# Auxeno/diamond-ppo

Measured on NVIDIA B200. Metric: ppo_update_samples_per_s, higher is better.
Workload: dtype f32

## Files before the change

diamond-ppo_b200/csrc/api.cu:

```cuda
#include "common.cuh"
#include "heads.cuh"
#include "optim.cuh"
#include "gemm_tc.cuh"

char g_dppo_create_error[512] = "";

extern "C" int dppo_version(void) { return DPPO_VERSION; }

extern "C" const char* dppo_last_error(dppo_ctx* ctx) { return ctx ? ctx->err : g_dppo_create_error; }

extern "C" int dppo_create(dppo_ctx** out, int device)
{
    if (!out) return 1;
    *out = nullptr;
    int count = 0;
    cudaError_t e = cudaGetDeviceCount(&count);
    if (e != cudaSuccess || count == 0) {
        snprintf(g_dppo_create_error, sizeof(g_dppo_create_error),
                 "dppo_create: no CUDA device (%s); libdppo has no CPU fallback", cudaGetErrorString(e));
        return 2;
    }
    if (device < 0 || device >= count) {
        snprintf(g_dppo_create_error, sizeof(g_dppo_create_error), "dppo_create: device %d out of range (%d devices)", device, count);
        return 3;
    }
    cudaDeviceProp prop;
    e = cudaGetDeviceProperties(&prop, device);
    if (e != cudaSuccess) {
        snprintf(g_dppo_create_error, sizeof(g_dppo_create_error), "dppo_create: %s", cudaGetErrorString(e));
        return 4;
    }
    if (prop.major != 10) {
        snprintf(g_dppo_create_error, sizeof(g_dppo_create_error),
                 "dppo_create: device %d is sm_%d%d; libdppo embeds sm_100a code only (B200) and has no fallback", device,
                 prop.major, prop.minor);
        return 5;
    }
    dppo_ctx* c = new dppo_ctx();
    c->device = device;
    c->sm_count = prop.multiProcessorCount;
    c->cc_major = prop.major;
    c->cc_minor = prop.minor;
    c->err[0] = 0;
    c->use_tensor_cores = 3;
    c->gae_variant = 0;
    c->gae_inputs_settled = 0;
    c->tc_debug = 0;
    c->row_sweep = 31;
    c->tc_prefetch = 0;
    c->draw_base = nullptr;
    c->rows_dev = nullptr;
    c->launch_count = 0;
    c->tm_cache = nullptr;
    c->tm_cache_free = nullptr;
    *out = c;
    return 0;
}

extern "C" int dppo_destroy(dppo_ctx* ctx)
{
    if (ctx && ctx->tm_cache && ctx->tm_cache_free) ctx->tm_cache_free(ctx->tm_cache);
    delete ctx;
    return 0;
}

extern "C" int dppo_set_option(dppo_ctx* ctx, const char* name, int value)
{
    if (!ctx || !name) return 1;
    if (!strcmp(name, "tensor_cores")) { ctx->use_tensor_cores = value != 0 ? 3 : 0; return 0; }
    if (!strcmp(name, "row_sweep")) { ctx->row_sweep = value & 31; return 0; }
    if (!strcmp(name, "tc_prefetch")) { ctx->tc_prefetch = value & 7; return 0; }
    if (!strcmp(name, "gae_variant")) { ctx->gae_variant = value; return 0; }
    if (!strcmp(name, "tc_debug")) {
#ifdef DPPO_TIMING_SWITCHES
        ctx->tc_debug = value;
        return 0;
#else
        DPPO_FAIL(ctx, "dppo_set_option: 'tc_debug' needs a library built with -DDPPO_TIMING_SWITCHES (timing experiments only)");
#endif
    }
    if (!strcmp(name, "gae_inputs_settled")) { ctx->gae_inputs_settled = value < 0 ? 0 : value > 2 ? 2 : value; return 0; }
    DPPO_FAIL(ctx, "dppo_set_option: unknown option '%s'", name);
}

extern "C" int64_t dppo_launch_count(dppo_ctx* ctx) { return ctx ? ctx->launch_count : 0; }

extern "C" int dppo_count_launches(dppo_ctx* ctx, int64_t n)
{
    if (!ctx) return 1;
    ctx->launch_count += n;
    return 0;
}

extern "C" int dppo_device_info(dppo_ctx* ctx, int* sm_count, int* cc_major, int* cc_minor)
{
    if (!ctx) return 1;
    if (sm_count) *sm_count = ctx->sm_count;
    if (cc_major) *cc_major = ctx->cc_major;
    if (cc_minor) *cc_minor = ctx->cc_minor;
    return 0;
}

extern "C" int dppo_mlp_layout_compute(const dppo_mlp_desc* d, dppo_mlp_layout* L)
{
    if (!d || !L || d->obs_dim < 1 || d->hidden < 1 || d->act_dim < 1) return 1;
    const int64_t D = d->obs_dim, H = d->hidden, A = d->act_dim;
    int64_t o = 0;
    auto take = [&](int64_t n) { const int64_t at = o; o += align_up(n, 4); return at; };
    L->w1 = take(H * D); L->b1 = take(H);
    L->w2 = take(H * H); L->b2 = take(H);
    L->w3 = take(2 * H * H); L->b3 = take(2 * H);
    L->wa = take(A * H); L->ba = take(A);
    L->wc = take(H); L->bc = take(1);
    L->log_std = d->continuous ? take(A) : -1;
    L->total = o;
    return 0;
}

namespace {

struct WImages {
    unsigned char *w1f, *w2f, *w3f, *w3b, *w2b;
    int64_t bytes;
};

WImages carve_images(const dppo_mlp_desc* d, char* base)
{
    const int64_t D = d->obs_dim, H = d->hidden;
    WImages w;
    int64_t o = 0;
    auto take = [&](int64_t bytes) { unsigned char* p = reinterpret_cast<unsigned char*>(base + o); o += align_up(bytes, 1024); return p; };
    w.w1f = take(dppo_tc_image_bytes((int)H, (int)D));
    w.w2f = take(dppo_tc_image_bytes((int)H, (int)H));
    w.w3f = take(dppo_tc_image_bytes((int)(2 * H), (int)H));
    w.w3b = take(dppo_tc_image_bytes((int)H, (int)(2 * H)));
    w.w2b = take(dppo_tc_image_bytes((int)H, (int)H));
    w.bytes = o;
    return w;
}

struct TrainWs {
    float *h1, *h2, *h3, *d3, *d2, *d1, *xg;
    float *p3, *p2, *p1, *c2, *c1, *hp;
    int s3, s2, s1, tiles2, tiles1, head_blocks, head_stride;
    int t3, t2, t1;
    bool multi;
    float *zd, *pa, *ca;
    int sa, tiles_a;
    int64_t img_off;
    int64_t bytes;
};

TrainWs carve_train(const dppo_mlp_desc* d, int64_t M, int sm_count, char* base, bool gemm_heads = false)
{
    dppo_ctx fake = {}; fake.sm_count = sm_count;
    const int64_t D = d->obs_dim, H = d->hidden, A = d->act_dim;
    TrainWs w;
    int64_t o = 0;
    auto take = [&](int64_t floats) { float* p = reinterpret_cast<float*>(base + o); o += align_up(floats * 4, 256); return p; };
    w.h1 = take(M * H); w.h2 = take(M * H); w.h3 = take(M * 2 * H);
    w.d3 = take(M * 2 * H); w.d2 = take(M * H); w.d1 = take(M * H);
    w.xg = take(M * D);
    w.s3 = dppo_wgrad_splits(&fake, M, (int)(2 * H), (int)H);
    w.s2 = dppo_wgrad_splits(&fake, M, (int)H, (int)H);
    w.s1 = dppo_wgrad_splits(&fake, M, (int)H, (int)D);
    w.t3 = dppo_tc2_wgrad_supported(M, (int)(2 * H), (int)H) ? dppo_tc2_wgrad_splits(&fake, M, (int)(2 * H), (int)H) : 0;
    w.t2 = dppo_tc2_wgrad_supported(M, (int)H, (int)H) ? dppo_tc2_wgrad_splits(&fake, M, (int)H, (int)H) : 0;
    w.t1 = dppo_tc2_wgrad_supported(M, (int)H, (int)D) ? dppo_tc2_wgrad_splits(&fake, M, (int)H, (int)D) : 0;
    w.multi = w.t3 > 0 && w.t2 > 0 && w.t1 > 0 && H % 256 == 0;
    if (w.multi) {
        const int n1s[3] = {(int)(2 * H), (int)H, (int)H}, n2s[3] = {(int)H, (int)H, (int)D};
        int sp[3];
        dppo_tc2_wgrad_multi_splits(&fake, M, 3, n1s, n2s, sp);
        w.t3 = sp[0]; w.t2 = sp[1]; w.t1 = sp[2];
    }
    auto mx = [](int a, int b) { return a > b ? a : b; };
    w.p3 = take((int64_t)mx(w.s3, w.t3) * 2 * H * H);
    w.p2 = take((int64_t)mx(w.s2, w.t2) * H * H);
    w.p1 = take((int64_t)mx(w.s1, w.t1) * H * D);
    w.tiles2 = dppo_gemm_row_tiles(M, (int)H);
    w.tiles1 = dppo_gemm_row_tiles(M, (int)H);
    const int cparts = mx(dppo_tc3_colsum_rows(&fake, M, (int)H), w.tiles2);
    w.c2 = take((int64_t)cparts * H);
    w.c1 = take((int64_t)cparts * H);
    w.zd = w.pa = w.ca = nullptr;
    w.sa = w.tiles_a = 0;
    if (gemm_heads) {
        w.zd = take(M * A);
        w.sa = dppo_wgrad_splits(&fake, M, (int)A, (int)H);
        w.pa = take((int64_t)w.sa * A * H);
        w.tiles_a = dppo_gemm_row_tiles(M, (int)H);
        w.ca = take((int64_t)w.tiles_a * H);
        w.head_blocks = wide_loss_blocks(&fake, M, (int)H, (int)A);
        w.head_stride = wide_offsets((int)H, (int)A).total;
    } else {
        w.head_blocks = head_train_blocks(&fake, M, (int)H, (int)A);
        w.head_stride = (int)align_up(head_partial_floats((int)H, (int)A), 4);
    }
    w.hp = take((int64_t)w.head_blocks * w.head_stride);
    o = align_up(o, 1024);
    w.img_off = o;
    o += carve_images(d, nullptr).bytes;
    w.bytes = o;
    return w;
}

int current_sm_count()
{
    int dev = 0, sms = 148;
    if (cudaGetDevice(&dev) == cudaSuccess) cudaDeviceGetAttribute(&sms, cudaDevAttrMultiProcessorCount, dev);
    return sms > 0 ? sms : 148;
}

}

extern "C" int64_t dppo_mlp_workspace_bytes(const dppo_mlp_desc* d, int64_t rows, int training)
{
    if (!d || rows <= 0) return 0;
    const int64_t H = d->hidden;
    if (!training)
        return align_up(rows * H * 4, 256) * 2 + align_up(rows * 2 * H * 4, 256) + align_up(rows * (int64_t)d->obs_dim * 4, 256) + 1024 +
               carve_images(d, nullptr).bytes;
    int sms = current_sm_count();
    if (sms < 148) sms = 148;
    return carve_train(d, rows, sms, nullptr).bytes;
}

extern "C" int dppo_mlp_fused_heads_supported(const dppo_mlp_desc* d)
{
    return d && head_train_supported(d->hidden, d->act_dim) ? 1 : 0;
}

static bool gemm_heads_in_bound(const dppo_mlp_desc* d)
{
    return d->hidden >= 1 && d->hidden <= DPPO_GEMM_HEADS_MAX_HIDDEN && d->act_dim >= 1 && d->act_dim <= DPPO_GEMM_HEADS_MAX_ACT;
}

extern "C" int64_t dppo_mlp_gemm_heads_workspace_bytes(const dppo_mlp_desc* d, int64_t rows)
{
    if (!d || rows <= 0 || d->obs_dim < 1 || !gemm_heads_in_bound(d)) return 0;
    int sms = current_sm_count();
    if (sms < 148) sms = 148;
    return carve_train(d, rows, sms, nullptr, true).bytes;
}

extern "C" int dppo_mlp_forward(dppo_ctx* ctx, const dppo_mlp_desc* d, const float* params, const float* obs,
                                const int32_t* idx, int64_t rows, int heads, float* head_out, float* values, void* ws,
                                int64_t ws_bytes, void* stream)
{
    if (!ctx) return 1;
    if (!d || !params || !obs || rows <= 0) DPPO_FAIL(ctx, "mlp_forward: bad arguments");
    if ((heads & 3) == 0) DPPO_FAIL(ctx, "mlp_forward: heads mask selects nothing");
    if ((heads & 1) && !head_out) DPPO_FAIL(ctx, "mlp_forward: head_out is null");
    if ((heads & 2) && !values) DPPO_FAIL(ctx, "mlp_forward: values is null");
    dppo_mlp_layout L;
    if (dppo_mlp_layout_compute(d, &L)) DPPO_FAIL(ctx, "mlp_forward: bad descriptor");
    const int D = d->obs_dim, H = d->hidden, A = d->act_dim;
    cudaStream_t st = (cudaStream_t)stream;
    const int64_t img_bytes = align_up(carve_images(d, nullptr).bytes, 1024);
    char* base0 = (char*)ws;
    char* aligned = reinterpret_cast<char*>((reinterpret_cast<uintptr_t>(base0) + 1023) & ~(uintptr_t)1023);
    const int64_t head_room = (aligned - base0) + img_bytes;
    const bool tc_on = ctx->use_tensor_cores && ws_bytes > head_room + 3 * 256;
    WImages img = carve_images(d, aligned);
    char* base = tc_on ? aligned + img_bytes : base0;
    const int64_t avail = tc_on ? ws_bytes - head_room : ws_bytes;
    const int64_t per_row = (int64_t)4 * H * 4 + (idx ? (int64_t)D * 4 : 0);
    int64_t chunk = (avail - 4 * 256) / per_row;
    if (chunk > rows) chunk = rows;
    if (chunk < 1) DPPO_FAIL(ctx, "mlp_forward: workspace too small (%lld bytes, need >= %lld per row)", (long long)ws_bytes, (long long)per_row);
    float* h1 = (float*)base;
    float* h2 = (float*)(base + align_up(chunk * H * 4, 256));
    float* h3 = (float*)(base + 2 * align_up(chunk * H * 4, 256));
    float* xg = (float*)(base + 2 * align_up(chunk * H * 4, 256) + align_up(chunk * 2 * H * 4, 256));
    const bool actor = heads & 1, critic = heads & 2;
    const int sweep = ctx->row_sweep;
    const int hint = (sweep & 8) ? 2 : 0;
    const int64_t w3off = actor ? 0 : (int64_t)H * H;
    const int b3off = actor ? 0 : H;
    const int n3 = (actor && critic) ? 2 * H : H;
    const int64_t first = rows < chunk ? rows : chunk;
    const bool tc1 = tc_on && dppo_tc3_gemm_supported(first, H, D), tc2 = tc_on && dppo_tc3_gemm_supported(first, H, H),
               tc3 = tc_on && dppo_tc3_gemm_supported(first, n3, H);
    {
        PrepJobs jobs;
        jobs.n = 0;
        jobs.gather = GatherJob{nullptr, nullptr, nullptr, 0, 0};
        auto job = [&](bool on, const float* W, int rows_w, int cols_w, unsigned char* im) {
            if (on) { jobs.job[jobs.n].W = W; jobs.job[jobs.n].rows_w = rows_w; jobs.job[jobs.n].cols_w = cols_w;
                      jobs.job[jobs.n].transpose = 0; jobs.job[jobs.n].n_tile = 0; jobs.job[jobs.n].img = im; ++jobs.n; }
        };
        job(tc1, params + L.w1, H, D, img.w1f);
        job(tc2, params + L.w2, H, H, img.w2f);
        job(tc3, params + L.w3 + w3off, n3, H, img.w3f);
        if (dppo_tc_prep_weights_multi(ctx, jobs, st)) return 1;
    }
    for (int64_t r0 = 0; r0 < rows; r0 += chunk) {
        const int64_t n = rows - r0 < chunk ? rows - r0 : chunk;
        const float* x = idx ? obs : obs + r0 * D;
        const int32_t* rowsel = idx ? idx + r0 : nullptr;
        if (tc1 && dppo_tc3_gemm_supported(n, H, D)) {
            if (rowsel) {
                if (dppo_gather_rows_f32(ctx, obs, rowsel, xg, n, D, stream)) return 1;
                x = xg;
            }
            if (dppo_tc3_gemm(ctx, DPPO_EPI_BIAS_TANH, x, D, img.w1f, params + L.b1, nullptr, 0, h1, H, nullptr, n, H, D, hint, st)) return 1;
        } else if (dppo_gemm_nt(ctx, DPPO_EPI_BIAS_TANH, x, D, rowsel, params + L.w1, D, params + L.b1, h1, H, n, H, D, st)) return 1;
        if (tc2 && dppo_tc3_gemm_supported(n, H, H)) {
            if (dppo_tc3_gemm(ctx, DPPO_EPI_BIAS_TANH, h1, H, img.w2f, params + L.b2, nullptr, 0, h2, H, nullptr, n, H, H, (sweep & 1) | hint, st)) return 1;
        } else if (dppo_gemm_nt(ctx, DPPO_EPI_BIAS_TANH, h1, H, nullptr, params + L.w2, H, params + L.b2, h2, H, n, H, H, st)) return 1;
        if (tc3 && dppo_tc3_gemm_supported(n, n3, H)) {
            if (dppo_tc3_gemm(ctx, DPPO_EPI_BIAS_TANH, h2, H, img.w3f, params + L.b3 + b3off, nullptr, 0, h3, n3, nullptr, n, n3, H, hint, st)) return 1;
        } else if (dppo_gemm_nt(ctx, DPPO_EPI_BIAS_TANH, h2, H, nullptr, params + L.w3 + w3off, H, params + L.b3 + b3off, h3, n3, n, n3, H, st)) return 1;
        const float* ha = actor ? h3 : nullptr;
        const float* hc = critic ? (actor ? h3 + H : h3) : nullptr;
        if (launch_heads_forward(ctx, ha, hc, n3, params + L.wa, params + L.ba, params + L.wc, params + L.bc,
                                 head_out ? head_out + r0 * A : nullptr, values ? values + r0 : nullptr, n, H, A, (sweep >> 1) & 1, st)) return 1;
    }
    return 0;
}

static int mlp_grad_minibatch_impl(dppo_ctx* ctx, const char* what, bool gemm_heads, const dppo_mlp_desc* d, const float* params,
                                   float* grads, const float* obs, const void* actions, const float* old_log_probs, const float* adv,
                                   const float* returns, const double* adv_stats, const int32_t* idx, int64_t M, const dppo_hyper* hy,
                                   float* losses, void* ws, int64_t ws_bytes, void* stream)
{
    if (!ctx) return 1;
    if (!d || !params || !grads || !obs || !actions || !old_log_probs || !adv || !returns || !hy || !ws)
        DPPO_FAIL(ctx, "%s: null argument", what);
    if (M <= 0) DPPO_FAIL(ctx, "%s: empty minibatch", what);
    if (hy->advantage_norm && (!adv_stats || hy->adv_count < 2)) DPPO_FAIL(ctx, "%s: advantage_norm needs adv_stats and adv_count >= 2", what);
    dppo_mlp_layout L;
    if (dppo_mlp_layout_compute(d, &L)) DPPO_FAIL(ctx, "%s: bad descriptor", what);
    if (gemm_heads && !gemm_heads_in_bound(d))
        DPPO_FAIL(ctx, "%s: hidden %d / %d actions outside the GEMM-head bound (hidden <= %d, 1..%d actions)", what, d->hidden, d->act_dim,
                  DPPO_GEMM_HEADS_MAX_HIDDEN, DPPO_GEMM_HEADS_MAX_ACT);
    const int D = d->obs_dim, H = d->hidden, A = d->act_dim;
    TrainWs w = carve_train(d, M, ctx->sm_count, (char*)ws, gemm_heads);
    if (w.bytes > ws_bytes) DPPO_FAIL(ctx, "%s: workspace too small (%lld < %lld)", what, (long long)ws_bytes, (long long)w.bytes);
    cudaStream_t st = (cudaStream_t)stream;
    const float inv_m = 1.0f / (float)(hy->loss_denominator > 0 ? hy->loss_denominator : M);

    char* img_base = reinterpret_cast<char*>((reinterpret_cast<uintptr_t>((char*)ws + w.img_off) + 1023) & ~(uintptr_t)1023);
    const bool img_fits = (img_base - (char*)ws) + carve_images(d, nullptr).bytes <= ws_bytes;
    const bool tc_on = ctx->use_tensor_cores && img_fits;
    WImages img = carve_images(d, img_base);
    const bool g1 = tc_on && dppo_tc3_gemm_supported(M, H, D), g2 = tc_on && dppo_tc3_gemm_supported(M, H, H),
               g3 = tc_on && dppo_tc3_gemm_supported(M, 2 * H, H), gb3 = tc_on && dppo_tc3_gemm_supported(M, H, 2 * H), gb2 = g2;
    const bool wg3 = tc_on && w.t3 > 0, wg2 = tc_on && w.t2 > 0, wg1 = tc_on && w.t1 > 0;
    const int sweep = ctx->row_sweep;
    const int hint = (sweep & 8) ? 2 : 0;
    const float* x1 = obs;
    const int32_t* x1_idx = idx;
    bool gather_pending = idx && (g1 || wg1);
    if (gather_pending) { x1 = w.xg; x1_idx = nullptr; }
    {
        PrepJobs jobs;
        jobs.n = 0;
        jobs.gather = GatherJob{nullptr, nullptr, nullptr, 0, 0};
        auto job = [&](bool on, const float* W, int rows_w, int cols_w, int transpose, unsigned char* im) {
            if (on) { jobs.job[jobs.n].W = W; jobs.job[jobs.n].rows_w = rows_w; jobs.job[jobs.n].cols_w = cols_w;
                      jobs.job[jobs.n].transpose = transpose; jobs.job[jobs.n].n_tile = 0; jobs.job[jobs.n].img = im; ++jobs.n; }
        };
        job(g1, params + L.w1, H, D, 0, img.w1f);
        job(g2, params + L.w2, H, H, 0, img.w2f);
        job(g3, params + L.w3, 2 * H, H, 0, img.w3f);
        job(gb3, params + L.w3, 2 * H, H, 1, img.w3b);
        job(gb2, params + L.w2, H, H, 1, img.w2b);
        if (gather_pending && D % 4 == 0 && (reinterpret_cast<uintptr_t>(obs) & 15u) == 0 && (reinterpret_cast<uintptr_t>(w.xg) & 15u) == 0) {
            jobs.gather = GatherJob{reinterpret_cast<const float4*>(obs), idx, reinterpret_cast<float4*>(w.xg), M, D / 4};
            gather_pending = false;
        }
        if (dppo_tc_prep_weights_multi(ctx, jobs, st)) return 1;
    }
    if (gather_pending && dppo_gather_rows_f32(ctx, obs, idx, w.xg, M, D, stream)) return 1;

    if (g1) {
        if (dppo_tc3_gemm(ctx, DPPO_EPI_BIAS_TANH, x1, D, img.w1f, params + L.b1, nullptr, 0, w.h1, H, nullptr, M, H, D, hint, st)) return 1;
    } else if (dppo_gemm_nt(ctx, DPPO_EPI_BIAS_TANH, x1, D, x1_idx, params + L.w1, D, params + L.b1, w.h1, H, M, H, D, st)) return 1;
    if (g2) {
        if (dppo_tc3_gemm(ctx, DPPO_EPI_BIAS_TANH, w.h1, H, img.w2f, params + L.b2, nullptr, 0, w.h2, H, nullptr, M, H, H, (sweep & 1) | hint, st)) return 1;
    } else if (dppo_gemm_nt(ctx, DPPO_EPI_BIAS_TANH, w.h1, H, nullptr, params + L.w2, H, params + L.b2, w.h2, H, M, H, H, st)) return 1;
    if (g3) {
        if (dppo_tc3_gemm(ctx, DPPO_EPI_BIAS_TANH, w.h2, H, img.w3f, params + L.b3, nullptr, 0, w.h3, 2 * H, nullptr, M, 2 * H, H, hint, st)) return 1;
    } else if (dppo_gemm_nt(ctx, DPPO_EPI_BIAS_TANH, w.h2, H, nullptr, params + L.w3, H, params + L.b3, w.h3, 2 * H, M, 2 * H, H, st)) return 1;

    if (!gemm_heads) {
        HeadTrainArgs ha;
        ha.h3 = w.h3; ha.d3 = w.d3;
        ha.wa = params + L.wa; ha.ba = params + L.ba; ha.wc = params + L.wc; ha.bc = params + L.bc;
        ha.log_std = d->continuous ? params + L.log_std : nullptr;
        ha.idx = idx;
        ha.actions_i = d->continuous ? nullptr : (const int32_t*)actions;
        ha.actions_f = d->continuous ? (const float*)actions : nullptr;
        ha.old_logp = old_log_probs; ha.adv = adv; ha.ret = returns;
        ha.adv_stats = adv_stats; ha.adv_count = hy->adv_count; ha.advantage_norm = hy->advantage_norm;
        ha.M = M; ha.H = H; ha.A = A;
        ha.clip = hy->ppo_clip; ha.vw = hy->value_loss_weight; ha.beta = hy->entropy_beta; ha.inv_m = inv_m;
        ha.partials = w.hp; ha.partial_stride = w.head_stride;
        ha.rev = (sweep >> 1) & 1; ha.keep_d3 = (sweep >> 2) & 1; ha.h3_first = (sweep >> 3) & 1;
        if (launch_head_train_kernel(ctx, ha, d->continuous, w.head_blocks, st)) return 1;
    } else {
        if (dppo_gemm_nt(ctx, DPPO_EPI_BIAS, w.h3, 2 * H, nullptr, params + L.wa, H, params + L.ba, w.zd, A, M, A, H, st)) return 1;
        WideLossArgs la = {};
        la.z = w.zd; la.dz = w.zd;
        la.log_std = d->continuous ? params + L.log_std : nullptr;
        la.h3 = w.h3; la.d3 = w.d3; la.wc = params + L.wc; la.bc = params + L.bc;
        la.idx = idx;
        la.actions_i = d->continuous ? nullptr : (const int32_t*)actions;
        la.actions_f = d->continuous ? (const float*)actions : nullptr;
        la.old_logp = old_log_probs; la.adv = adv; la.ret = returns;
        la.adv_stats = adv_stats; la.adv_count = hy->adv_count; la.advantage_norm = hy->advantage_norm;
        la.M = M; la.H = H; la.A = A;
        la.clip = hy->ppo_clip; la.vw = hy->value_loss_weight; la.beta = hy->entropy_beta; la.inv_m = inv_m;
        la.partials = w.hp; la.partial_stride = w.head_stride;
        if (launch_wide_loss_train(ctx, la, d->continuous, w.head_blocks, st)) return 1;
        if (dppo_gemm_nn_tanh_bwd(ctx, w.zd, A, params + L.wa, H, w.h3, 2 * H, w.d3, 2 * H, w.ca, M, H, A, st)) return 1;
        if (dppo_wgrad(ctx, w.zd, A, w.h3, 2 * H, nullptr, w.pa, w.sa, M, A, H, st)) return 1;
    }

    int tiles2 = w.tiles2, tiles1 = w.tiles1;
    if (gb3) {
        tiles2 = dppo_tc3_colsum_parts(ctx, M, H);
        if (dppo_tc3_gemm(ctx, DPPO_EPI_TANH_BWD, w.d3, 2 * H, img.w3b, nullptr, w.h2, H, w.d2, H, w.c2, M, H, 2 * H, hint, st)) return 1;
    } else if (dppo_gemm_nn_tanh_bwd(ctx, w.d3, 2 * H, params + L.w3, H, w.h2, H, w.d2, H, w.c2, M, H, 2 * H, st)) return 1;
    if (gb2) {
        tiles1 = dppo_tc3_colsum_parts(ctx, M, H);
        if (dppo_tc3_gemm(ctx, DPPO_EPI_TANH_BWD, w.d2, H, img.w2b, nullptr, w.h1, H, w.d1, H, w.c1, M, H, H, sweep & 1, st)) return 1;
    } else if (dppo_gemm_nn_tanh_bwd(ctx, w.d2, H, params + L.w2, H, w.h1, H, w.d1, H, w.c1, M, H, H, st)) return 1;
    const int n3p = wg3 ? w.t3 : w.s3, n2p = wg2 ? w.t2 : w.s2, n1p = wg1 ? w.t1 : w.s1;
    if (w.multi && wg3 && wg2 && wg1) {
        const float* Ds[3] = {w.d3, w.d2, w.d1};
        const float* Hs[3] = {w.h2, w.h1, x1};
        float* Ps[3] = {w.p3, w.p2, w.p1};
        const int ldds[3] = {2 * H, H, H}, ldhs[3] = {H, H, D}, sps[3] = {w.t3, w.t2, w.t1}, n1s[3] = {2 * H, H, H}, n2s[3] = {H, H, D};
        if (dppo_tc2_wgrad_multi(ctx, 3, Ds, ldds, Hs, ldhs, Ps, sps, M, n1s, n2s, st)) return 1;
    } else {
    if (wg3) {
        if (dppo_tc2_wgrad(ctx, w.d3, 2 * H, w.h2, H, w.p3, w.t3, M, 2 * H, H, st)) return 1;
    } else if (dppo_wgrad(ctx, w.d3, 2 * H, w.h2, H, nullptr, w.p3, w.s3, M, 2 * H, H, st)) return 1;
    if (wg2) {
        if (dppo_tc2_wgrad(ctx, w.d2, H, w.h1, H, w.p2, w.t2, M, H, H, st)) return 1;
    } else if (dppo_wgrad(ctx, w.d2, H, w.h1, H, nullptr, w.p2, w.s2, M, H, H, st)) return 1;
    if (wg1) {
        if (dppo_tc2_wgrad(ctx, w.d1, H, x1, D, w.p1, w.t1, M, H, D, st)) return 1;
    } else if (dppo_wgrad(ctx, w.d1, H, x1, D, x1_idx, w.p1, w.s1, M, H, D, st)) return 1;
    }

    GradSegTable tab;
    int n = 0;
    auto seg = [&](int64_t dst, int64_t count, const float* src, int64_t stride, int nparts) {
        tab.seg[n].dst = dst; tab.seg[n].count = count; tab.seg[n].src = src; tab.seg[n].stride = stride;
        tab.seg[n].nparts = nparts; tab.seg[n].pad = 0; ++n;
    };
    seg(L.w1, (int64_t)H * D, w.p1, (int64_t)H * D, n1p);
    seg(L.b1, H, w.c1, H, tiles1);
    seg(L.w2, (int64_t)H * H, w.p2, (int64_t)H * H, n2p);
    seg(L.b2, H, w.c2, H, tiles2);
    seg(L.w3, (int64_t)2 * H * H, w.p3, (int64_t)2 * H * H, n3p);
    int off_dba, off_dwc, off_dbc, off_dls, off_loss;
    if (!gemm_heads) {
        const HeadOffsets ho = head_offsets(H, A);
        off_dba = ho.dba; off_dwc = ho.dwc; off_dbc = ho.dbc; off_dls = ho.dls; off_loss = ho.loss;
        seg(L.b3, 2 * H, w.hp + ho.b3, w.head_stride, w.head_blocks);
        seg(L.wa, (int64_t)A * H, w.hp, w.head_stride, w.head_blocks);
    } else {
        const WideOffsets wo = wide_offsets(H, A);
        off_dba = wo.dba; off_dwc = wo.dwc; off_dbc = wo.dbc; off_dls = wo.dls; off_loss = 0;
        seg(L.b3, H, w.ca, H, w.tiles_a);
        seg(L.b3 + H, H, w.hp + wo.db3, w.head_stride, w.head_blocks);
        seg(L.wa, (int64_t)A * H, w.pa, (int64_t)A * H, w.sa);
    }
    seg(L.ba, A, w.hp + off_dba, w.head_stride, w.head_blocks);
    seg(L.wc, H, w.hp + off_dwc, w.head_stride, w.head_blocks);
    seg(L.bc, 1, w.hp + off_dbc, w.head_stride, w.head_blocks);
    if (d->continuous) seg(L.log_std, A, w.hp + off_dls, w.head_stride, w.head_blocks);
    tab.nseg = n;
    return launch_grad_reduce(ctx, tab, grads, L.total, w.hp + off_loss, w.head_blocks, w.head_stride, hy->value_loss_weight,
                              hy->entropy_beta, inv_m, losses, hy->grad_sumsq, st);
}

extern "C" int dppo_mlp_grad_minibatch(dppo_ctx* ctx, const dppo_mlp_desc* d, const float* params, float* grads,
                                       const float* obs, const void* actions, const float* old_log_probs, const float* adv,
                                       const float* returns, const double* adv_stats, const int32_t* idx, int64_t M,
                                       const dppo_hyper* hy, float* losses, void* ws, int64_t ws_bytes, void* stream)
{
    return mlp_grad_minibatch_impl(ctx, "mlp_grad_minibatch", false, d, params, grads, obs, actions, old_log_probs, adv, returns,
                                   adv_stats, idx, M, hy, losses, ws, ws_bytes, stream);
}

extern "C" int dppo_mlp_grad_minibatch_gemm_heads(dppo_ctx* ctx, const dppo_mlp_desc* d, const float* params, float* grads,
                                                  const float* obs, const void* actions, const float* old_log_probs, const float* adv,
                                                  const float* returns, const double* adv_stats, const int32_t* idx, int64_t M,
                                                  const dppo_hyper* hy, float* losses, void* ws, int64_t ws_bytes, void* stream)
{
    return mlp_grad_minibatch_impl(ctx, "mlp_grad_minibatch_gemm_heads", true, d, params, grads, obs, actions, old_log_probs, adv,
                                   returns, adv_stats, idx, M, hy, losses, ws, ws_bytes, stream);
}

namespace {

__global__ void __launch_bounds__(256)
next_value_plan_kernel(const float* __restrict__ terms, const float* __restrict__ truncs, const float* __restrict__ values, int T, int N,
                       float* __restrict__ next_values, int32_t* __restrict__ idx, int* __restrict__ count)
{
    const int64_t B = (int64_t)T * N;
    const int lane = threadIdx.x & 31;
    for (int64_t base = (int64_t)blockIdx.x * blockDim.x; base < B; base += (int64_t)gridDim.x * blockDim.x) {
        const int64_t i = base + threadIdx.x;
        bool need = false;
        if (i < B) {
            need = i >= B - N || terms[i] != 0.0f || truncs[i] != 0.0f;
            if (!need) next_values[i] = values[i + N];
        }
        const unsigned ballot = __ballot_sync(0xffffffffu, need);
        int start = 0;
        if (lane == 0 && ballot) start = atomicAdd(count, __popc(ballot));
        start = __shfl_sync(0xffffffffu, start, 0);
        if (need) idx[start + __popc(ballot & ((1u << lane) - 1u))] = (int32_t)i;
    }
}

__global__ void __launch_bounds__(256)
scatter_values_kernel(const float* __restrict__ src, const int32_t* __restrict__ idx, const int* __restrict__ count, float* __restrict__ dst)
{
    const int n = *count;
    for (int i = blockIdx.x * blockDim.x + threadIdx.x; i < n; i += gridDim.x * blockDim.x) dst[idx[i]] = src[i];
}

struct NextWs { int* count; int32_t* idx; float *xg, *h1, *h2, *h3, *tmp; int64_t img_off, bytes; };

NextWs carve_next(const dppo_mlp_desc* d, int64_t B, char* base)
{
    NextWs w;
    int64_t o = 0;
// ... 126 lines not shown
```

diamond-ppo_b200/csrc/common.cuh:

```cuda
#pragma once
#include <cuda_runtime.h>
#include <stdint.h>
#include <stdio.h>
#include <string.h>

#include "dppo.h"

struct dppo_ctx {
    int device;
    int sm_count;
    int cc_major, cc_minor;
    char err[512];
    int use_tensor_cores;
    int gae_variant;
    int gae_inputs_settled;
    long long launch_count;
    int row_sweep;
    int tc_prefetch;
    int tc_debug;
    const unsigned long long* draw_base;
    const int* rows_dev;
    void* tm_cache;
    void (*tm_cache_free)(void*);
};

extern char g_dppo_create_error[512];

#define DPPO_FAIL(ctx, ...)                                   \
    do {                                                      \
        if (ctx) snprintf((ctx)->err, sizeof((ctx)->err), __VA_ARGS__); \
        return 1;                                             \
    } while (0)

#define DPPO_CHECK_LAUNCH(ctx, what)                                                        \
    do {                                                                                    \
        cudaError_t e_ = cudaGetLastError();                                                \
        if (e_ != cudaSuccess) DPPO_FAIL(ctx, "%s: %s", what, cudaGetErrorString(e_));      \
        ++(ctx)->launch_count;                                                              \
    } while (0)

#ifdef DPPO_TIMING_SWITCHES
#define DPPO_DBG(mask, bit) (((mask) & (bit)) != 0)
#else
#define DPPO_DBG(mask, bit) false
#endif

static inline int64_t align_up(int64_t x, int64_t a) { return (x + a - 1) / a * a; }

#define DPPO_PDL_ENTER()                                                    \
    do {                                                                    \
        asm volatile("griddepcontrol.launch_dependents;" ::: "memory");     \
        asm volatile("griddepcontrol.wait;" ::: "memory");                  \
    } while (0)

template <typename... KArgs, typename... Args>
static inline cudaError_t dppo_launch_pdl_if(bool on, void (*kern)(KArgs...), dim3 grid, dim3 block, size_t smem, cudaStream_t st, Args&&... args)
{
    cudaLaunchConfig_t lc = {};
    lc.gridDim = grid; lc.blockDim = block; lc.dynamicSmemBytes = smem; lc.stream = st;
    cudaLaunchAttribute attr[1];
    attr[0].id = cudaLaunchAttributeProgrammaticStreamSerialization;
    attr[0].val.programmaticStreamSerializationAllowed = 1;
    lc.attrs = attr;
    lc.numAttrs = on ? 1 : 0;
    return cudaLaunchKernelEx(&lc, kern, static_cast<KArgs>(args)...);
}
template <typename... KArgs, typename... Args>
static inline cudaError_t dppo_launch_pdl(dppo_ctx* ctx, void (*kern)(KArgs...), dim3 grid, dim3 block, size_t smem, cudaStream_t st,
                                          Args&&... args)
{
    return dppo_launch_pdl_if(DPPO_DBG(ctx->tc_debug, 512), kern, grid, block, smem, st, static_cast<Args&&>(args)...);
}

__device__ __forceinline__ uint64_t l2_policy_evict_first()
{
    uint64_t p;
    asm volatile("createpolicy.fractional.L2::evict_first.b64 %0, 1.0;" : "=l"(p));
    return p;
}
__device__ __forceinline__ float4 ldg_l2_hint(const float4* p, uint64_t policy)
{
    float4 v;
    asm("ld.global.nc.L2::cache_hint.v4.f32 {%0, %1, %2, %3}, [%4], %5;" : "=f"(v.x), "=f"(v.y), "=f"(v.z), "=f"(v.w) : "l"(p), "l"(policy));
    return v;
}

__device__ __forceinline__ float warp_sum(float v) {
#pragma unroll
    for (int o = 16; o > 0; o >>= 1) v += __shfl_xor_sync(0xffffffffu, v, o);
    return v;
}
__device__ __forceinline__ double warp_sum_d(double v) {
#pragma unroll
    for (int o = 16; o > 0; o >>= 1) v += __shfl_xor_sync(0xffffffffu, v, o);
    return v;
}
__device__ __forceinline__ float warp_max(float v) {
#pragma unroll
    for (int o = 16; o > 0; o >>= 1) v = fmaxf(v, __shfl_xor_sync(0xffffffffu, v, o));
    return v;
}

enum { DPPO_EPI_BIAS = 0, DPPO_EPI_BIAS_TANH = 1, DPPO_EPI_TANH_BWD = 2, DPPO_EPI_NONE = 3 };
int dppo_gemm_nt(dppo_ctx* ctx, int epi, const float* A, int lda, const int32_t* a_rows, const float* B, int ldb,
                 const float* bias, float* C, int ldc, int64_t M, int N, int K, cudaStream_t st);
int dppo_gemm_nn_tanh_bwd(dppo_ctx* ctx, const float* A, int lda, const float* B, int ldb, const float* Hact, int ldh,
                          float* C, int ldc, float* colsum, int64_t M, int N, int K, cudaStream_t st);
int dppo_gemm_nn(dppo_ctx* ctx, const float* A, int lda, const float* B, int ldb, float* C, int ldc, int64_t M, int N, int K,
                 cudaStream_t st);
int dppo_gemm_row_tiles(int64_t M, int N);
int dppo_wgrad_splits(dppo_ctx* ctx, int64_t M, int N1, int N2);
int dppo_wgrad(dppo_ctx* ctx, const float* A, int lda, const float* B, int ldb, const int32_t* b_rows,
               float* partials, int splits, int64_t M, int N1, int N2, cudaStream_t st);
```

diamond-ppo_b200/csrc/gemm_tc.cuh:

```cuda
#pragma once
#include "common.cuh"

int dppo_tc_n_tile(int N);
int64_t dppo_tc_image_bytes(int N, int K);
int dppo_tc_prep_weights(dppo_ctx* ctx, const float* W, int rows_w, int cols_w, int transpose, unsigned char* img, cudaStream_t st);
struct PrepJob { const float* W; int rows_w, cols_w, transpose, n_tile; unsigned char* img; };
struct GatherJob { const float4* src; const int32_t* idx; float4* dst; int64_t rows; int row_vec; };
struct PrepJobs { PrepJob job[8]; int n; GatherJob gather; };
int dppo_tc_prep_weights_multi(dppo_ctx* ctx, PrepJobs jobs, cudaStream_t st);

bool dppo_tc2_wgrad_supported(int64_t M, int N1, int N2);
int dppo_tc2_wgrad_splits(dppo_ctx* ctx, int64_t M, int N1, int N2);
int dppo_tc2_wgrad(dppo_ctx* ctx, const float* Dm, int ldd, const float* Hm, int ldh, float* partials, int splits, int64_t M, int N1,
                   int N2, cudaStream_t st);
void dppo_tc2_wgrad_multi_splits(dppo_ctx* ctx, int64_t M, int n, const int* N1, const int* N2, int* splits_out);
int dppo_tc2_wgrad_multi(dppo_ctx* ctx, int n, const float* const* Dm, const int* ldd, const float* const* Hm, const int* ldh,
                         float* const* partials, const int* splits, int64_t M, const int* N1, const int* N2, cudaStream_t st);

bool dppo_tc3_gemm_supported(int64_t M, int N, int K);
int dppo_tc3_colsum_parts(dppo_ctx* ctx, int64_t M, int N);
int dppo_tc3_colsum_rows(dppo_ctx* ctx, int64_t M, int N);
int dppo_tc3_gemm(dppo_ctx* ctx, int epi, const float* A, int lda, const unsigned char* Wimg, const float* bias, const float* Hact,
                  int ldh, float* C, int ldc, float* colsum, int64_t M, int N, int K, int rev, cudaStream_t st);
```

Measured before the change: 107.9 million.

## Fuse first two trunk layers into one 2-CTA tcgen05 kernel keeping h1 in TMEM

```diff
diff --git a/diamond-ppo_b200/csrc/api.cu b/diamond-ppo_b200/csrc/api.cu
--- a/diamond-ppo_b200/csrc/api.cu
+++ b/diamond-ppo_b200/csrc/api.cu
@@ -48,6 +48,7 @@
     c->tc_debug = 0;
     c->row_sweep = 31;
     c->tc_prefetch = 0;
+    c->trunk_fusion = 1;
     c->draw_base = nullptr;
     c->rows_dev = nullptr;
     c->launch_count = 0;
@@ -70,6 +71,7 @@
     if (!strcmp(name, "tensor_cores")) { ctx->use_tensor_cores = value != 0 ? 3 : 0; return 0; }
     if (!strcmp(name, "row_sweep")) { ctx->row_sweep = value & 31; return 0; }
     if (!strcmp(name, "tc_prefetch")) { ctx->tc_prefetch = value & 7; return 0; }
+    if (!strcmp(name, "trunk_fusion")) { ctx->trunk_fusion = value & 3; return 0; }
     if (!strcmp(name, "gae_variant")) { ctx->gae_variant = value; return 0; }
     if (!strcmp(name, "tc_debug")) {
 #ifdef DPPO_TIMING_SWITCHES
@@ -299,16 +301,24 @@
         const int64_t n = rows - r0 < chunk ? rows - r0 : chunk;
         const float* x = idx ? obs : obs + r0 * D;
         const int32_t* rowsel = idx ? idx + r0 : nullptr;
-        if (tc1 && dppo_tc3_gemm_supported(n, H, D)) {
+        if (tc1 && tc2 && (ctx->trunk_fusion & 1) && dppo_trunk12_supported(ctx, n, H, D)) {
             if (rowsel) {
                 if (dppo_gather_rows_f32(ctx, obs, rowsel, xg, n, D, stream)) return 1;
                 x = xg;
             }
-            if (dppo_tc3_gemm(ctx, DPPO_EPI_BIAS_TANH, x, D, img.w1f, params + L.b1, nullptr, 0, h1, H, nullptr, n, H, D, hint, st)) return 1;
-        } else if (dppo_gemm_nt(ctx, DPPO_EPI_BIAS_TANH, x, D, rowsel, params + L.w1, D, params + L.b1, h1, H, n, H, D, st)) return 1;
-        if (tc2 && dppo_tc3_gemm_supported(n, H, H)) {
-            if (dppo_tc3_gemm(ctx, DPPO_EPI_BIAS_TANH, h1, H, img.w2f, params + L.b2, nullptr, 0, h2, H, nullptr, n, H, H, (sweep & 1) | hint, st)) return 1;
-        } else if (dppo_gemm_nt(ctx, DPPO_EPI_BIAS_TANH, h1, H, nullptr, params + L.w2, H, params + L.b2, h2, H, n, H, H, st)) return 1;
+            if (dppo_trunk12(ctx, x, D, img.w1f, params + L.b1, img.w2f, params + L.b2, nullptr, h2, n, D, (sweep & 1) | hint, st)) return 1;
+        } else {
+            if (tc1 && dppo_tc3_gemm_supported(n, H, D)) {
+                if (rowsel) {
+                    if (dppo_gather_rows_f32(ctx, obs, rowsel, xg, n, D, stream)) return 1;
+                    x = xg;
+                }
+                if (dppo_tc3_gemm(ctx, DPPO_EPI_BIAS_TANH, x, D, img.w1f, params + L.b1, nullptr, 0, h1, H, nullptr, n, H, D, hint, st)) return 1;
+            } else if (dppo_gemm_nt(ctx, DPPO_EPI_BIAS_TANH, x, D, rowsel, params + L.w1, D, params + L.b1, h1, H, n, H, D, st)) return 1;
+            if (tc2 && dppo_tc3_gemm_supported(n, H, H)) {
+                if (dppo_tc3_gemm(ctx, DPPO_EPI_BIAS_TANH, h1, H, img.w2f, params + L.b2, nullptr, 0, h2, H, nullptr, n, H, H, (sweep & 1) | hint, st)) return 1;
+            } else if (dppo_gemm_nt(ctx, DPPO_EPI_BIAS_TANH, h1, H, nullptr, params + L.w2, H, params + L.b2, h2, H, n, H, H, st)) return 1;
+        }
         if (tc3 && dppo_tc3_gemm_supported(n, n3, H)) {
             if (dppo_tc3_gemm(ctx, DPPO_EPI_BIAS_TANH, h2, H, img.w3f, params + L.b3 + b3off, nullptr, 0, h3, n3, nullptr, n, n3, H, hint, st)) return 1;
         } else if (dppo_gemm_nt(ctx, DPPO_EPI_BIAS_TANH, h2, H, nullptr, params + L.w3 + w3off, H, params + L.b3 + b3off, h3, n3, n, n3, H, st)) return 1;
@@ -375,12 +385,16 @@
     }
     if (gather_pending && dppo_gather_rows_f32(ctx, obs, idx, w.xg, M, D, stream)) return 1;
 
-    if (g1) {
-        if (dppo_tc3_gemm(ctx, DPPO_EPI_BIAS_TANH, x1, D, img.w1f, params + L.b1, nullptr, 0, w.h1, H, nullptr, M, H, D, hint, st)) return 1;
-    } else if (dppo_gemm_nt(ctx, DPPO_EPI_BIAS_TANH, x1, D, x1_idx, params + L.w1, D, params + L.b1, w.h1, H, M, H, D, st)) return 1;
-    if (g2) {
-        if (dppo_tc3_gemm(ctx, DPPO_EPI_BIAS_TANH, w.h1, H, img.w2f, params + L.b2, nullptr, 0, w.h2, H, nullptr, M, H, H, (sweep & 1) | hint, st)) return 1;
-    } else if (dppo_gemm_nt(ctx, DPPO_EPI_BIAS_TANH, w.h1, H, nullptr, params + L.w2, H, params + L.b2, w.h2, H, M, H, H, st)) return 1;
+    if (g1 && g2 && (ctx->trunk_fusion & 2) && dppo_trunk12_supported(ctx, M, H, D)) {
+        if (dppo_trunk12(ctx, x1, D, img.w1f, params + L.b1, img.w2f, params + L.b2, w.h1, w.h2, M, D, (sweep & 1) | hint, st)) return 1;
+    } else {
+        if (g1) {
+            if (dppo_tc3_gemm(ctx, DPPO_EPI_BIAS_TANH, x1, D, img.w1f, params + L.b1, nullptr, 0, w.h1, H, nullptr, M, H, D, hint, st)) return 1;
+        } else if (dppo_gemm_nt(ctx, DPPO_EPI_BIAS_TANH, x1, D, x1_idx, params + L.w1, D, params + L.b1, w.h1, H, M, H, D, st)) return 1;
+        if (g2) {
+            if (dppo_tc3_gemm(ctx, DPPO_EPI_BIAS_TANH, w.h1, H, img.w2f, params + L.b2, nullptr, 0, w.h2, H, nullptr, M, H, H, (sweep & 1) | hint, st)) return 1;
+        } else if (dppo_gemm_nt(ctx, DPPO_EPI_BIAS_TANH, w.h1, H, nullptr, params + L.w2, H, params + L.b2, w.h2, H, M, H, H, st)) return 1;
+    }
     if (g3) {
         if (dppo_tc3_gemm(ctx, DPPO_EPI_BIAS_TANH, w.h2, H, img.w3f, params + L.b3, nullptr, 0, w.h3, 2 * H, nullptr, M, 2 * H, H, hint, st)) return 1;
     } else if (dppo_gemm_nt(ctx, DPPO_EPI_BIAS_TANH, w.h2, H, nullptr, params + L.w3, H, params + L.b3, w.h3, 2 * H, M, 2 * H, H, st)) return 1;
diff --git a/diamond-ppo_b200/csrc/common.cuh b/diamond-ppo_b200/csrc/common.cuh
--- a/diamond-ppo_b200/csrc/common.cuh
+++ b/diamond-ppo_b200/csrc/common.cuh
@@ -17,6 +17,7 @@
     long long launch_count;
     int row_sweep;
     int tc_prefetch;
+    int trunk_fusion;
     int tc_debug;
     const unsigned long long* draw_base;
     const int* rows_dev;
diff --git a/diamond-ppo_b200/csrc/gemm_tc.cuh b/diamond-ppo_b200/csrc/gemm_tc.cuh
--- a/diamond-ppo_b200/csrc/gemm_tc.cuh
+++ b/diamond-ppo_b200/csrc/gemm_tc.cuh
@@ -22,3 +22,7 @@
 int dppo_tc3_colsum_rows(dppo_ctx* ctx, int64_t M, int N);
 int dppo_tc3_gemm(dppo_ctx* ctx, int epi, const float* A, int lda, const unsigned char* Wimg, const float* bias, const float* Hact,
                   int ldh, float* C, int ldc, float* colsum, int64_t M, int N, int K, int rev, cudaStream_t st);
+
+bool dppo_trunk12_supported(dppo_ctx* ctx, int64_t M, int H, int D);
+int dppo_trunk12(dppo_ctx* ctx, const float* x, int ldx, const unsigned char* w1img, const float* b1, const unsigned char* w2img,
+                 const float* b2, float* h1, float* h2, int64_t M, int D, int rev, cudaStream_t st);
diff --git a/diamond-ppo_b200/csrc/trunk_tc3.cu b/diamond-ppo_b200/csrc/trunk_tc3.cu
--- /dev/null
+++ b/diamond-ppo_b200/csrc/trunk_tc3.cu
@@ -0,0 +1,293 @@
+#include <cuda.h>
+
+#include "tc_common.cuh"
+#include "gemm_tc.cuh"
+
+using namespace tc;
+
+namespace {
+
+constexpr int THREADS = 576;
+constexpr int W_PROD = 0, W_MMA = 1, W_E1 = 2, N_E1 = 8, W_E2 = 10, N_E2 = 8;
+constexpr int HID = 256;
+constexpr int KC = 16;
+constexpr int BM = 128;
+constexpr int A_IMG = BM * KC * 4;
+constexpr int B_HALF = (HID / 2) * KC * 4;
+constexpr int B_IMG = HID * KC * 4;
+constexpr int STAGE = 2 * A_IMG + 2 * B_HALF;
+constexpr int STAGES = 6;
+constexpr int L2_CHUNKS = HID / KC;
+constexpr int STG_BLK = 32 * 128;
+constexpr size_t SMEM = (size_t)STAGES * STAGE + (size_t)N_E2 * STG_BLK + 1024;
+
+__device__ __forceinline__ void tmem_ld16_issue(uint32_t taddr, uint32_t (&r)[16])
+{
+    asm volatile(
+        "tcgen05.ld.sync.aligned.32x32b.x16.b32 "
+        "{%0, %1, %2, %3, %4, %5, %6, %7, %8, %9, %10, %11, %12, %13, %14, %15}, [%16];"
+        : "=r"(r[0]), "=r"(r[1]), "=r"(r[2]), "=r"(r[3]), "=r"(r[4]), "=r"(r[5]), "=r"(r[6]), "=r"(r[7]), "=r"(r[8]), "=r"(r[9]),
+          "=r"(r[10]), "=r"(r[11]), "=r"(r[12]), "=r"(r[13]), "=r"(r[14]), "=r"(r[15])
+        : "r"(taddr));
+}
+__device__ __forceinline__ void tmem_ld16_wait(uint32_t (&r)[16])
+{
+    asm volatile("tcgen05.wait::ld.sync.aligned;"
+                 : "+r"(r[0]), "+r"(r[1]), "+r"(r[2]), "+r"(r[3]), "+r"(r[4]), "+r"(r[5]), "+r"(r[6]), "+r"(r[7]), "+r"(r[8]), "+r"(r[9]),
+                   "+r"(r[10]), "+r"(r[11]), "+r"(r[12]), "+r"(r[13]), "+r"(r[14]), "+r"(r[15])
+                 :
+                 : "memory");
+}
+
+__global__ void __cluster_dims__(2, 1, 1) __launch_bounds__(THREADS, 1)
+trunk12_kernel(const __grid_constant__ CUtensorMap tmX, const __grid_constant__ CUtensorMap tmH1, const __grid_constant__ CUtensorMap tmH2,
+               const unsigned char* __restrict__ w1img, const float* __restrict__ b1, const unsigned char* __restrict__ w2img,
+               const float* __restrict__ b2, int D, int blocks, int rev, int store_h1)
+{
+    extern __shared__ unsigned char dyn_raw[];
+    __shared__ __align__(8) uint64_t full[STAGES], ready[STAGES], empty[STAGES], xfull, xempty, yfull, yempty;
+    __shared__ uint32_t s_tmem;
+
+    unsigned char* dyn = reinterpret_cast<unsigned char*>((reinterpret_cast<uintptr_t>(dyn_raw) + 1023) & ~(uintptr_t)1023);
+    const int tid = threadIdx.x, warp = tid >> 5, lane = tid & 31;
+    const uint32_t rank = cluster_ctarank();
+    const int cluster_id = blockIdx.x >> 1, n_clusters = gridDim.x >> 1;
+    const bool in_first = (rev & 2) != 0;
+    rev &= 1;
+    const int c1 = D / KC;
+    const int cpb = c1 + L2_CHUNKS;
+    const int n_my = blocks / n_clusters + (cluster_id < blocks % n_clusters ? 1 : 0);
+    auto block_of = [&](int i) { const int t = i * n_clusters + cluster_id; return rev ? blocks - 1 - t : t; };
+
+    if (tid == 0) {
+#pragma unroll
+        for (int s = 0; s < STAGES; ++s) { mbar_init(&full[s], 1); mbar_init(&ready[s], 2 * 4); mbar_init(&empty[s], 1 + 4); }
+        mbar_init(&xfull, 1); mbar_init(&xempty, 2 * N_E1);
+        mbar_init(&yfull, 1); mbar_init(&yempty, 2 * N_E2);
+        fence_mbar_init();
+    }
+    if (warp == W_MMA) tmem_alloc2(&s_tmem, 512);
+    fence_before();
+    cluster_sync();
+    fence_after();
+    const uint32_t tmem = s_tmem;
+    DPPO_PDL_ENTER();
+
+    if (warp == W_PROD) {
+        if (lane == 0) {
+            tma_prefetch_desc(&tmX);
+            const uint64_t pol = l2_policy_evict_first();
+            const int64_t w_off = (int64_t)rank * (HID / 2) * KC * 4;
+            int s = 0;
+            uint32_t ph = 0;
+            for (int i = 0; i < n_my; ++i) {
+                const int m0 = block_of(i) * 2 * BM + (int)rank * BM;
+                for (int j = 0; j < cpb; ++j) {
+                    mbar_wait(&empty[s], ph ^ 1);
+                    unsigned char* st = dyn + s * STAGE;
+                    const unsigned char* w;
+                    if (j < c1) {
+                        mbar_expect_tx(&full[s], (uint32_t)(A_IMG + 2 * B_HALF));
+                        if (in_first) tma_load_2d_hint(st, &tmX, j * KC, m0, &full[s], pol);
+                        else tma_load_2d(st, &tmX, j * KC, m0, &full[s]);
+                        w = w1img + w_off + (int64_t)j * 2 * B_IMG;
+                    } else {
+                        mbar_expect_tx(&full[s], (uint32_t)(2 * B_HALF));
+                        w = w2img + w_off + (int64_t)(j - c1) * 2 * B_IMG;
+                    }
+                    bulk_copy_g2s(st + 2 * A_IMG, w, (uint32_t)B_HALF, &full[s]);
+                    bulk_copy_g2s(st + 2 * A_IMG + B_HALF, w + B_IMG, (uint32_t)B_HALF, &full[s]);
+                    if (++s == STAGES) { s = 0; ph ^= 1; }
+                }
+            }
+        }
+        __syncwarp();
+    } else if (warp == W_MMA) {
+        if (rank == 0 && lane == 0) {
+            const uint32_t idesc = idesc_tf32(2 * BM, HID, 0, 0);
+            int s = 0;
+            uint32_t ph = 0;
+            auto chunk = [&](uint32_t d, bool first) {
+                mbar_wait(&ready[s], ph);
+                fence_after();
+                const uint32_t a_hi = smem_u32(dyn + s * STAGE), a_lo = a_hi + A_IMG;
+                const uint32_t b_hi = a_hi + 2 * A_IMG, b_lo = b_hi + B_HALF;
+#pragma unroll
+                for (int ks = 0; ks < KC / 8; ++ks) {
+                    const uint32_t ko = ks * 32;
+                    umma_tf32_2cta(d, desc_k_sw64(a_hi + ko), desc_k_sw64(b_lo + ko), idesc, (first && ks == 0) ? 0u : 1u);
+                    umma_tf32_2cta(d, desc_k_sw64(a_lo + ko), desc_k_sw64(b_hi + ko), idesc, 1u);
+                    umma_tf32_2cta(d, desc_k_sw64(a_hi + ko), desc_k_sw64(b_hi + ko), idesc, 1u);
+                }
+                umma_commit_2cta(&empty[s], 3);
+                if (++s == STAGES) { s = 0; ph ^= 1; }
+            };
+            for (uint32_t i = 0; i < (uint32_t)n_my; ++i) {
+                mbar_wait(&xempty, (i & 1) ^ 1);
+                fence_after();
+                for (int j = 0; j < c1; ++j) chunk(tmem, j == 0);
+                umma_commit_2cta(&xfull, 3);
+                mbar_wait(&yempty, (i & 1) ^ 1);
+                fence_after();
+                for (int k = 0; k < L2_CHUNKS; ++k) chunk(tmem + HID, k == 0);
+                umma_commit_2cta(&yfull, 3);
+            }
+        }
+        __syncwarp();
+    } else if (warp < W_E2) {
+        const int ew = warp - W_E1;
+        const int set = ew >> 2, q = warp & 3;
+        const int ct = (ew & 3) * 32 + lane;
+        const int r = q * 32 + lane;
+        const uint32_t row_off = (uint32_t)r * 64, sw = (uint32_t)((r >> 1) & 3);
+        if (lane == 0 && store_h1) tma_prefetch_desc(&tmH1);
+        int s = 0, prev_s = -1;
+        uint32_t ph = 0;
+        int g = 0;
+        for (int i = 0; i < n_my; ++i) {
+            const int m0 = block_of(i) * 2 * BM + (int)rank * BM;
+            for (int j = 0; j < cpb; ++j, ++g) {
+                if ((g & 1) == set) {
+                    mbar_wait(&full[s], ph);
+                    const uint32_t st = smem_u32(dyn + s * STAGE);
+                    if (j < c1) {
+                        constexpr int PER = A_IMG / 16 / 128;
+                        if (lane == 0 && prev_s >= 0) { bulk_wait_read<0>(); mbar_arrive(&empty[prev_s]); }
+                        float4 x[PER];
+#pragma unroll
+                        for (int p = 0; p < PER; ++p) x[p] = lds128(st + ct * 16 + p * 128 * 16);
+#pragma unroll
+                        for (int p = 0; p < PER; ++p) sts128(st + A_IMG + ct * 16 + p * 128 * 16, lo_of_trunc_x4(x[p]));
+                        fence_proxy_async();
+                        __syncwarp();
+                    } else {
+                        const int k = j - c1;
+                        mbar_wait(&xfull, (uint32_t)(i & 1));
+                        fence_after();
+                        uint32_t a[16];
+                        tmem_ld16_issue(tmem + ((uint32_t)(q * 32) << 16) + (uint32_t)(k * KC), a);
+                        float4 bb[4];
+#pragma unroll
+                        for (int p = 0; p < 4; ++p) bb[p] = __ldg(reinterpret_cast<const float4*>(b1 + k * KC) + p);
+                        tmem_ld16_wait(a);
+                        if (k >= L2_CHUNKS - 2) {
+                            fence_before();
+                            __syncwarp();
+                            if (lane == 0) mbar_arrive_cluster(mapa(smem_u32(&xempty), 0));
+                        }
+                        if (lane == 0 && prev_s >= 0) { bulk_wait_read<0>(); mbar_arrive(&empty[prev_s]); }
+                        __syncwarp();
+#pragma unroll
+                        for (int p = 0; p < 4; ++p) {
+                            float4 h;
+                            h.x = tanh_rational(__uint_as_float(a[4 * p]) + bb[p].x);
+                            h.y = tanh_rational(__uint_as_float(a[4 * p + 1]) + bb[p].y);
+                            h.z = tanh_rational(__uint_as_float(a[4 * p + 2]) + bb[p].z);
+                            h.w = tanh_rational(__uint_as_float(a[4 * p + 3]) + bb[p].w);
+                            const uint32_t o = row_off + ((((uint32_t)p) ^ sw) << 4);
+                            sts128(st + o, h);
+                            sts128(st + A_IMG + o, lo_of_trunc_x4(h));
+                        }
+                        fence_proxy_async();
+                        __syncwarp();
+                        if (lane == 0 && store_h1) {
+                            tma_store_2d(&tmH1, k * KC, m0 + q * 32, st + (uint32_t)q * 32 * 64);
+                            bulk_commit();
+                        }
+                    }
+                    if (lane == 0) mbar_arrive_cluster(mapa(smem_u32(&ready[s]), 0));
+                    prev_s = s;
+                }
+                if (++s == STAGES) { s = 0; ph ^= 1; }
+            }
+        }
+        if (lane == 0) bulk_wait<0>();
+        __syncwarp();
+    } else {
+        const int ew = warp - W_E2;
+        const int q = warp & 3, grp = ew >> 2;
+        const uint32_t stg = smem_u32(dyn + STAGES * STAGE) + (uint32_t)ew * STG_BLK;
+        const uint32_t row_off = (uint32_t)lane * 128, sw = (uint32_t)(lane & 7);
+        constexpr int NCOLS = HID / 2, NBLK = NCOLS / 32;
+        if (lane == 0) tma_prefetch_desc(&tmH2);
+        for (uint32_t i = 0; i < (uint32_t)n_my; ++i) {
+            const int m0 = block_of((int)i) * 2 * BM + (int)rank * BM + q * 32;
+            const int col0 = grp * NCOLS;
+            mbar_wait(&yfull, i & 1);
+            fence_after();
+            for (int k = 0; k < NBLK; ++k) {
+                const int n = col0 + k * 32;
+                uint32_t rr[32];
+                tmem_ld32_issue(tmem + HID + ((uint32_t)(q * 32) << 16) + (uint32_t)n, rr);
+                float4 aux[8];
+#pragma unroll
+                for (int j = 0; j < 8; ++j) aux[j] = __ldg(reinterpret_cast<const float4*>(b2 + n) + j);
+                tmem_ld32_wait(rr);
+                if (k == NBLK - 1) {
+                    fence_before();
+                    __syncwarp();
+                    if (lane == 0) mbar_arrive_cluster(mapa(smem_u32(&yempty), 0));
+                }
+                float v[32];
+#pragma unroll
+                for (int j = 0; j < 8; ++j) {
+                    v[4 * j] = tanh_rational(__uint_as_float(rr[4 * j]) + aux[j].x);
+                    v[4 * j + 1] = tanh_rational(__uint_as_float(rr[4 * j + 1]) + aux[j].y);
+                    v[4 * j + 2] = tanh_rational(__uint_as_float(rr[4 * j + 2]) + aux[j].z);
+                    v[4 * j + 3] = tanh_rational(__uint_as_float(rr[4 * j + 3]) + aux[j].w);
+                }
+                if (lane == 0) bulk_wait_read<0>();
+                __syncwarp();
+#pragma unroll
+                for (int j = 0; j < 8; ++j)
+                    sts128(stg + row_off + ((((uint32_t)j) ^ sw) << 4), make_float4(v[4 * j], v[4 * j + 1], v[4 * j + 2], v[4 * j + 3]));
+                fence_proxy_async();
+                __syncwarp();
+                if (lane == 0) {
+                    tma_store_2d(&tmH2, n, m0, stg);
+                    bulk_commit();
+                }
+            }
+        }
+        if (lane == 0) bulk_wait<0>();
+        __syncwarp();
+    }
+
+    fence_before();
+    cluster_sync();
+    if (warp == W_MMA) {
+        fence_after();
+        tmem_dealloc2(tmem, 512);
+    }
+}
+
+bool al16(const void* p) { return (reinterpret_cast<uintptr_t>(p) & 15u) == 0; }
+
+}
+
+bool dppo_trunk12_supported(dppo_ctx* ctx, int64_t M, int H, int D)
+{
+    const int64_t blocks = (M + 2 * BM - 1) / (2 * BM);
+    return ctx->rows_dev == nullptr && H == HID && D >= KC && D % KC == 0 && M < (int64_t)1 << 31 &&
+           ctx->sm_count >= 2 && blocks >= ctx->sm_count / 2;
+}
+
+int dppo_trunk12(dppo_ctx* ctx, const float* x, int ldx, const unsigned char* w1img, const float* b1, const unsigned char* w2img,
+                 const float* b2, float* h1, float* h2, int64_t M, int D, int rev, cudaStream_t st)
+{
+    if (!dppo_trunk12_supported(ctx, M, HID, D)) DPPO_FAIL(ctx, "trunk12: unsupported shape M=%lld D=%d", (long long)M, D);
+    if (ldx % 4 != 0 || !al16(x) || !al16(w1img) || !al16(w2img) || !al16(b1) || !al16(b2) || !al16(h2) || (h1 && !al16(h1)))
+        DPPO_FAIL(ctx, "trunk12: operands must be 16-byte aligned with row pitches multiple of 4 floats");
+    CUtensorMap tmX, tmH1, tmH2;
+    if (!dppo_make_tensor_map_2d(&tmX, x, M, D, ldx, KC, BM, 2) || !dppo_make_tensor_map_2d(&tmH2, h2, M, HID, HID, 32, 32, 3) ||
+        (h1 && !dppo_make_tensor_map_2d(&tmH1, h1, M, HID, HID, KC, 32, 2)))
+        DPPO_FAIL(ctx, "trunk12: cuTensorMapEncodeTiled failed");
+    if (!h1) tmH1 = tmH2;
+    const int blocks = (int)((M + 2 * BM - 1) / (2 * BM));
+    const int grid = 2 * (ctx->sm_count / 2);
+    cudaFuncSetAttribute(trunk12_kernel, cudaFuncAttributeMaxDynamicSharedMemorySize, (int)SMEM);
+    dppo_launch_pdl_if(true, trunk12_kernel, dim3(grid), dim3(THREADS), SMEM, st, tmX, tmH1, tmH2, w1img, b1, w2img, b2, D, blocks, rev,
+                       h1 ? 1 : 0);
+    DPPO_CHECK_LAUNCH(ctx, "trunk12_kernel");
+    return 0;
+}
diff --git a/profiles/trunk_fusion_ab.py b/profiles/trunk_fusion_ab.py
--- /dev/null
+++ b/profiles/trunk_fusion_ab.py
@@ -0,0 +1,138 @@
+#!/usr/bin/env python
+import argparse
+import json
+import os
+import subprocess
+import sys
+import threading
+import time
+
+import numpy as np
+import torch
+
+ROOT = os.path.dirname(os.path.dirname(os.path.abspath(__file__)))
+for p in (ROOT, os.path.join(ROOT, "diamond-ppo_b200")):
+    if p not in sys.path:
+        sys.path.insert(0, p)
+
+import bench
+
+T, N_ENVS, D, H, A, E, MB = bench.T, bench.N_ENVS, bench.D, bench.H, bench.A, bench.E, bench.MB
+MASKS = (0, 1, 3)
+
+
+def card():
+    q = subprocess.run(["nvidia-smi", "--query-gpu=name,power.limit", "--format=csv,noheader", "-i", str(torch.cuda.current_device())],
+                       capture_output=True, text=True).stdout.strip()
+    return q or torch.cuda.get_device_name()
+
+
+class Clocks(threading.Thread):
+    def __init__(self):
+        super().__init__(daemon=True)
+        self.stop, self.sm = threading.Event(), []
+
+    def run(self):
+        while not self.stop.is_set():
+            q = subprocess.run(["nvidia-smi", "--query-gpu=clocks.sm", "--format=csv,noheader,nounits", "-i",
+                                str(torch.cuda.current_device())], capture_output=True, text=True).stdout.strip()
+            try:
+                self.sm.append(float(q))
+            except ValueError:
+                pass
+            time.sleep(0.2)
+
+
+def trunk_forward_us(ctx, fm, flat, obs_sets, ws_sets, reps=24):
+    M = obs_sets[0].shape[0]
+    val = torch.empty(M, device="cuda")
+    for o, w in zip(obs_sets, ws_sets):
+        ctx.mlp_forward(fm.desc, flat, o, M, 2, None, val, w)
+    torch.cuda.synchronize()
+    e0, e1 = torch.cuda.Event(enable_timing=True), torch.cuda.Event(enable_timing=True)
+    e0.record()
+    for i in range(reps):
+        ctx.mlp_forward(fm.desc, flat, obs_sets[i % len(obs_sets)], M, 2, None, val, ws_sets[i % len(ws_sets)])
+    e1.record()
+    torch.cuda.synchronize()
+    return e0.elapsed_time(e1) * 1e3 / reps
+
+
+def main():
+    ap = argparse.ArgumentParser()
+    ap.add_argument("--rounds", type=int, default=5)
+    ap.add_argument("--steps", type=int, default=10)
+    ap.add_argument("--out", default=None)
+    args = ap.parse_args()
+    from diamond import PPO, PPOConfig, envs, _native
+    from diamond.agents import RolloutBuffer
+    ctx = _native.get_context(0)
+
+    def env_fn(n):
+        return envs.BatchedSyntheticVectorEnv(n, D, A)
+    env_fn.vectorized = True
+
+    host = bench.synth_host_rollout(1)
+    agents, bufs = [], []
+    for k in MASKS:
+        ctx.set_option("trunk_fusion", k)
+        cfg = PPOConfig(num_envs=N_ENVS, rollout_steps=T, network_hidden_dim=H, num_epochs=E, num_minibatches=MB, verbose=False,
+                        total_steps=T * N_ENVS * 1000, seed=7)
+        ag = PPO(env_fn, cfg)
+        buf = RolloutBuffer(ctx, T, N_ENVS, D, 1, False, ag.device)
+        buf.load_host(*host)
+        for _ in range(3):
+            ag.learn(buf)
+        agents.append(ag); bufs.append(buf)
+    torch.cuda.synchronize()
+
+    fm = agents[0].engine.fm
+    flat = agents[0].engine.P
+    M = T * N_ENVS // MB
+    g = torch.Generator(device="cuda").manual_seed(3)
+    obs_sets = [torch.randn(M, D, device="cuda", generator=g) for _ in range(4)]
+    ws_sets = [torch.empty(ctx.mlp_workspace_bytes(fm.desc, M, False) // 4 + 512, device="cuda") for _ in range(4)]
+
+    clocks = Clocks()
+    clocks.start()
+    rows = []
+    for r in range(args.rounds):
+        for j, k in enumerate(MASKS):
+            ctx.set_option("trunk_fusion", k)
+            ag, buf = agents[j], bufs[j]
+            evs = []
+            e0, e1 = torch.cuda.Event(enable_timing=True), torch.cuda.Event(enable_timing=True)
+            torch.cuda.synchronize()
+            e0.record()
+            for _ in range(args.steps):
+                ev = {}
+                ag.learn(buf, events=ev)
+                evs.append(ev)
+            e1.record()
+            torch.cuda.synchronize()
+            row = dict(round=r, trunk_fusion=k, ms_per_learn=e0.elapsed_time(e1) / args.steps,
+                       update_us_per_step=float(np.mean([v["gae_end"].elapsed_time(v["update_end"]) for v in evs])) * 1e3 / (E * MB),
+                       prepass_ms=float(np.mean([v["start"].elapsed_time(v["prepass_end"]) for v in evs])),
+                       critic_forward_us=trunk_forward_us(ctx, fm, flat, obs_sets, ws_sets))
+            rows.append(row)
+            print(json.dumps(row), flush=True)
+    clocks.stop.set()
+    clocks.join()
+    ctx.set_option("trunk_fusion", 1)
+
+    summary = {"card": card(), "median_sm_clock_mhz": float(np.median(clocks.sm)) if clocks.sm else None}
+    for key in ("ms_per_learn", "update_us_per_step", "prepass_ms", "critic_forward_us"):
+        a = [x[key] for x in rows if x["trunk_fusion"] == 0]
+        summary[key] = {"mask0_median": float(np.median(a))}
+        for k in MASKS[1:]:
+            b = [x[key] for x in rows if x["trunk_fusion"] == k]
+            summary[key][f"mask{k}"] = {"median": float(np.median(b)), "gain_pct": 100.0 * (np.median(a) - np.median(b)) / np.median(a),
+                                        "faster_every_round": bool(all(y < x for x, y in zip(a, b)))}
+    print(json.dumps(summary), flush=True)
+    if args.out:
+        os.makedirs(args.out, exist_ok=True)
+        json.dump({"rounds": rows, "summary": summary}, open(os.path.join(args.out, "trunk_fusion_ab.json"), "w"), indent=1)
+
+
+if __name__ == "__main__":
+    main()
```

Result: no change. 108.6 million (median of 6 runs) (+0.6%).
